# tomasjakab/imm

Measured on AMD Instinct MI355X. Metric: training images/sec at 128x128 K=10, higher is better.
Workload: dtype bf16; 1 GPU; BASELINE configs[1] (N>1: configs[2]): CelebA-shape 128x128 K=10 IMM training step (fwd + VGG16 perceptual loss + bwd + clip + Adam), batch 32 per GPU; global_batch=32, image_size=128, n_maps=10, parallelism=dp1, hip_graph=True, weights=seeded random init; synthetic VGG16 (vgg16.caffemodel.h5 unavailable offline)

## Files before the change

### imm_amd/csrc/conv_wgrad_halo.hip

```cpp
#include "conv_common.h"
#include "conv_dispatch.h"
#include <stdlib.h>
#include <string.h>

typedef __attribute__((ext_vector_type(4))) short s16x4_t;
typedef __attribute__((address_space(3))) s16x4_t lds_s16x4_t;

#ifndef IMM_WH_ABLATE
#define IMM_WH_ABLATE 0
#endif
#define WH_PH 8
#define WH_PW 16
#define WH_HROWS(KH) (WH_PH + (KH) - 1)
#define WH_HCOLS(KW) (WH_PW + (KW) - 1)
#define WH_HP(KH, KW) ((WH_HROWS(KH) * WH_HCOLS(KW) + 63) / 64 * 64)
#define WH_S2_PW 17
#define WH_S2_PP 160
#define WH_S2_HP 640

template <int C8>
__device__ __forceinline__ int wh_swzx(int x) { return C8 == 8 ? ((((x >> 1) & 1) | (((x >> 3) & 1) << 1)) << 1) : (((x >> 3) & 1) << 1); }

struct WgradHaloArgs {
  const uint16_t* x; const uint16_t* dy; float* slab;
  int batch, h, w, ldx, lddy, co, kpad, ci_total;
  int n_patches, patches_x, patches_y;
  int nsplit, nci, nco;
  uint32_t x_bytes, dy_bytes;
  const float* nol_scale; const float* nol_shift; int nol_relu;
};

template <typename ET, int CI, int CO, int NS, int KH = 3, int KW = 3, int ST = 1>
__device__ __forceinline__ void conv_wgrad_halo_body(const WgradHaloArgs& a, const int bx, const int G, const int by, const int bz) {
  static_assert(ST == 1 || (ST == 2 && KH == 3 && KW == 3), "stride 2: 3x3 only");
  constexpr int NTAP = KH * KW, PT = (KH - 1) / 2, PL = (KW - 1) / 2;
  constexpr int WH_HW = WH_HCOLS(KW), HPIX = WH_HROWS(KH) * WH_HCOLS(KW), WH_HP_ = ST == 2 ? WH_S2_HP : WH_HP(KH, KW);
  constexpr int XC8 = CI / 8, YC8 = CO / 8;
  constexpr int NCT = CI / 16, NNT = CO / 16;
  constexpr int WC = NCT, WN = 4 / WC;
  constexpr int TNT = NNT / WN;
  static_assert(WC * WN == 4 && TNT >= 1, "tile split");
  constexpr int X_PIX_PER_DMA = 64 / XC8, Y_PIX_PER_DMA = 64 / YC8;
  constexpr int X_DMA = WH_HP_ / X_PIX_PER_DMA, Y_DMA = 128 / Y_PIX_PER_DMA;
  constexpr int X_BYTES = WH_HP_ * CI * 2, Y_BYTES = 128 * CO * 2, STAGE = X_BYTES + Y_BYTES;
  constexpr int LPP = X_DMA / 4 + Y_DMA / 4;
  static_assert(X_DMA % 4 == 0 && Y_DMA % 4 == 0 && NS >= 2 && (NS - 2) * LPP < 64, "uniform per-wave DMA count");
  extern __shared__ __attribute__((aligned(16))) uint4 smem[];
  const bool nol = a.nol_scale != nullptr;
  float* coef = (float*)((char*)smem + NS * STAGE);

  const int tid = threadIdx.x, lane = tid & 63, wid = tid >> 6;
  const int wc = wid % WC, wn = wid / WC;
  const int ci0 = by * CI, co0 = bz * CO;
  const u32x4_t xr = buffer_rsrc(a.x, a.x_bytes), yr = buffer_rsrc(a.dy, a.dy_bytes);
  const uint32_t lds_base = (uint32_t)(size_t)(lds_void_t*)smem;
  const int per_img = a.patches_x * a.patches_y;

  constexpr int XU = X_DMA / 4, YU = Y_DMA / 4;
  int x_iy[XU], x_ix[XU];
  int x_rel[XU];
  int x_sc[XU];
  uint32_t y_rel[YU];
  const int w_in = ST * a.w, h_in = ST * a.h;
#pragma unroll
  for (int u = 0; u < XU; ++u) {
    const int hp = (wid + 4 * u) * X_PIX_PER_DMA + lane / XC8;
    int iy, ix, col;
    bool valid;
    if constexpr (ST == 2) {
      const int plane = hp / WH_S2_PP, rem = hp - plane * WH_S2_PP;
      const int pi = rem / WH_S2_PW, pj = rem - pi * WH_S2_PW;
      iy = 2 * pi + (plane >> 1); ix = 2 * pj + (plane & 1);
      valid = rem < 9 * WH_S2_PW;
      col = pj;
    } else {
      const int hy = hp / WH_HW, hx = hp - hy * WH_HW;
      iy = hy - PT; ix = hx - PL;
      valid = hp < HPIX;
      col = hx;
    }
    const int sc = (lane % XC8) ^ wh_swzx<XC8>(col);
    x_iy[u] = valid ? iy : (1 << 24);
    x_ix[u] = ix;
    x_rel[u] = ((iy * w_in + ix) * a.ldx + ci0) * 2 + sc * 16;
    x_sc[u] = sc;
  }
  if (nol && tid < CI) {
    coef[(tid >> 3) * 16 + (tid & 7)] = a.nol_scale[ci0 + tid];
    coef[(tid >> 3) * 16 + 8 + (tid & 7)] = a.nol_shift[ci0 + tid];
  }
#pragma unroll
  for (int u = 0; u < YU; ++u) {
    const int p = (wid + 4 * u) * Y_PIX_PER_DMA + lane / YC8;
    const int ty = p >> 4, tx = p & 15;
    const int sc = (lane % YC8) ^ wh_swzx<YC8>(tx);
    y_rel[u] = (uint32_t)(((ty * a.w + tx) * a.lddy + co0) * 2 + sc * 16);
  }

  auto issue = [&](int patch, int stage) {
    const int img = patch / per_img, pr = patch - img * per_img;
    const int y0 = (pr / a.patches_x) * WH_PH, x0 = (pr % a.patches_x) * WH_PW;
    const uint32_t xs = (uint32_t)(img * h_in * w_in) * (uint32_t)(a.ldx * 2);
    const uint32_t ys = (uint32_t)(img * a.h * a.w) * (uint32_t)(a.lddy * 2) + (uint32_t)((y0 * a.w + x0) * a.lddy * 2);
    const int py = ST * y0, px = ST * x0;
    const int poff = (py * w_in + px) * a.ldx * 2;
    const uint32_t lds_stage = lds_base + (uint32_t)(stage * STAGE + wid * 1024);
#pragma unroll
    for (int u = 0; u < XU; ++u) {
      const bool ok = ((unsigned)(py + x_iy[u]) < (unsigned)h_in) && ((unsigned)(px + x_ix[u]) < (unsigned)w_in);
      const uint32_t vo = ok ? (uint32_t)(x_rel[u] + poff) : BUFFER_OOB;
      lds_dma16(xr, __builtin_amdgcn_readfirstlane(lds_stage + (uint32_t)(u * 4096)), vo, xs);
    }
#pragma unroll
    for (int u = 0; u < YU; ++u)
      lds_dma16(yr, __builtin_amdgcn_readfirstlane(lds_stage + (uint32_t)(X_BYTES + u * 4096)), y_rel[u], ys);
  };

  f32x4_t acc[NTAP][TNT];
#pragma unroll
  for (int t = 0; t < NTAP; ++t)
#pragma unroll
    for (int j = 0; j < TNT; ++j) acc[t][j] = f32x4_t{0.f, 0.f, 0.f, 0.f};

  const int i16 = lane & 15, g = lane >> 4;
  const int k_row = g >> 1, k_x = (g & 1) * 8 + (i16 >> 2), ch4 = (i16 & 3) * 4;
  const char* lds_c = (const char*)smem;
  constexpr int KXE = ST == 2 ? 2 : KW;
  const int lx = k_row * (ST == 2 ? WH_S2_PW : WH_HW) + k_x, ly = k_row * WH_PW + k_x;
  uint32_t xb[KXE][2], yb[TNT][2];
#pragma unroll
  for (int e = 0; e < KXE; ++e)
#pragma unroll
    for (int h = 0; h < 2; ++h)
      xb[e][h] = (uint32_t)((lx * XC8 + (((wc * 16 + ch4) >> 3) ^ wh_swzx<XC8>(k_x + e + 4 * h))) * 16 + (ch4 & 4) * 2);
#pragma unroll
  for (int j = 0; j < TNT; ++j)
#pragma unroll
    for (int h = 0; h < 2; ++h)
      yb[j][h] = (uint32_t)(X_BYTES + (ly * YC8 + (((((wn * TNT + j) * 16) + ch4) >> 3) ^ wh_swzx<YC8>(k_x + 4 * h))) * 16 + (ch4 & 4) * 2);

  uint4 af_keep = make_uint4(0, 0, 0, 0);
  const int n_mine = (bx < a.n_patches) ? (a.n_patches - bx + G - 1) / G : 0;
#pragma unroll
  for (int t = 0; t < NS - 1; ++t)
    if (t < n_mine) issue(bx + t * G, t);
  int stage = 0;
  for (int it = 0; it < n_mine; ++it) {
    constexpr int ABL = IMM_WH_ABLATE;
    if (!(ABL & 16) || it == 0) {
      if (it + NS - 2 < n_mine) wait_vmcnt<(NS - 2) * LPP>();
      else wait_vmcnt<0>();
      if (nol) wait_lgkmcnt0();
      __builtin_amdgcn_s_barrier();
    }
    if (it + NS - 1 < n_mine && !(ABL & 1)) {
      int ns = stage + NS - 1; if (ns >= NS) ns -= NS;
      issue(bx + (it + NS - 1) * G, ns);
    }
    const char* Xl = lds_c + stage * STAGE;
    if (nol) {
      const int patch_ = bx + it * G;
      const int img_ = patch_ / per_img, pr_ = patch_ - img_ * per_img;
      const int py_ = ST * (pr_ / a.patches_x) * WH_PH, px_ = ST * (pr_ % a.patches_x) * WH_PW;
      char* Xw = (char*)smem + stage * STAGE + wid * 1024 + lane * 16;
      const bool nrelu = a.nol_relu != 0;
#pragma unroll
      for (int u = 0; u < XU; ++u) {
        if (((unsigned)(py_ + x_iy[u]) < (unsigned)h_in) && ((unsigned)(px_ + x_ix[u]) < (unsigned)w_in)) {
          uint4* slot = (uint4*)(Xw + u * 4096);
          float f[8];
          unpack8<ET>(*slot, f);
          const float4* cf = (const float4*)(coef + x_sc[u] * 16);
          const float4 s0 = cf[0], s1 = cf[1], h0 = cf[2], h1 = cf[3];
          const float sc[8] = {s0.x, s0.y, s0.z, s0.w, s1.x, s1.y, s1.z, s1.w};
          const float sh[8] = {h0.x, h0.y, h0.z, h0.w, h1.x, h1.y, h1.z, h1.w};
#pragma unroll
          for (int e = 0; e < 8; ++e) {
            f[e] = f[e] * sc[e] + sh[e];
            if (nrelu) f[e] = fmaxf(f[e], 0.f);
          }
          *slot = pack8<ET>(f);
        }
      }
      wait_lgkmcnt0();
      __builtin_amdgcn_s_barrier();
    }

    uint4 bfr[4][TNT];
    if (!(ABL & 4) || it == 0)
#pragma unroll
    for (int ks = 0; ks < 4; ++ks)
#pragma unroll
      for (int j = 0; j < TNT; ++j) {
        const s16x4_t lo = __builtin_amdgcn_ds_read_tr16_b64_v4i16((lds_s16x4_t*)(Xl + yb[j][0] + ks * 32 * YC8 * 16));
        const s16x4_t hi = __builtin_amdgcn_ds_read_tr16_b64_v4i16((lds_s16x4_t*)(Xl + yb[j][1] + (ks * 32 + 4) * YC8 * 16));
        const uint2 l2 = __builtin_bit_cast(uint2, lo), h2 = __builtin_bit_cast(uint2, hi);
        bfr[ks][j] = make_uint4(l2.x, l2.y, h2.x, h2.y);
      }
#pragma unroll
    for (int tap = 0; tap < NTAP; ++tap) {
      const int ky = tap / KW, kx = tap % KW;
#pragma unroll
      for (int ks = 0; ks < 4; ++ks) {
        const int e = ST == 2 ? (kx >> 1) : kx;
        const int cp = ST == 2 ? ((ky & 1) * 2 + (kx & 1)) * WH_S2_PP + (ks * 2 + (ky >> 1)) * WH_S2_PW + (kx >> 1)
                               : (ks * 2 + ky) * WH_HW + kx;
        uint4 af;
        if (!(ABL & 2) || (it == 0 && tap == 0 && ks == 0)) {
          const s16x4_t lo = __builtin_amdgcn_ds_read_tr16_b64_v4i16((lds_s16x4_t*)(Xl + xb[e][0] + cp * XC8 * 16));
          const s16x4_t hi = __builtin_amdgcn_ds_read_tr16_b64_v4i16((lds_s16x4_t*)(Xl + xb[e][1] + (cp + 4) * XC8 * 16));
          const uint2 l2 = __builtin_bit_cast(uint2, lo), h2 = __builtin_bit_cast(uint2, hi);
          af = make_uint4(l2.x, l2.y, h2.x, h2.y);
          af_keep = af;
        } else af = af_keep;
        if (!(ABL & 8))
#pragma unroll
        for (int j = 0; j < TNT; ++j) acc[tap][j] = ET::mfma(bfr[ks][j], af, acc[tap][j]);
      }
    }
    if (++stage == NS) stage = 0;
  }

  float* out = a.slab + (int64_t)bx * a.kpad * a.co;
#pragma unroll
  for (int tap = 0; tap < NTAP; ++tap) {
    const int kk = tap * a.ci_total + ci0 + wc * 16 + (lane & 15);
#pragma unroll
    for (int j = 0; j < TNT; ++j) {
      const int n = co0 + (wn * TNT + j) * 16 + 4 * (lane >> 4);
      float* op = out + (int64_t)kk * a.co + n;
      if (IMM_WH_ABLATE & 32) {
        if (acc[tap][j][0] == 123456.789f) op[0] = acc[tap][j][1] + acc[tap][j][2] + acc[tap][j][3];
      } else if (n + 3 < a.co && (a.co & 3) == 0) {
        *(float4*)op = make_float4(acc[tap][j][0], acc[tap][j][1], acc[tap][j][2], acc[tap][j][3]);
      } else {
#pragma unroll
        for (int r = 0; r < 4; ++r) if (n + r < a.co) op[r] = acc[tap][j][r];
      }
    }
  }
}

template <typename ET, int CI, int CO, int NS, int KH = 3, int KW = 3, int ST = 1>
__global__ __launch_bounds__(256) void conv_wgrad_halo_kernel(const WgradHaloArgs a) {
  conv_wgrad_halo_body<ET, CI, CO, NS, KH, KW, ST>(a, blockIdx.x, gridDim.x, blockIdx.y, blockIdx.z);
}

template <typename ET, int CI, int CO, int NS, int KH = 3, int KW = 3, int ST = 1>
__global__ __launch_bounds__(256) void conv_wgrad_halo_multi_kernel(const WgradHaloArgs* __restrict__ tab,
                                                                    const int* __restrict__ first, int n) {
  const int b = blockIdx.x;
  int g = 0;
  while (g + 1 < n && b >= first[g + 1]) ++g;
  const WgradHaloArgs a = tab[g];
  int r = b - first[g];
  const int bx = r % a.nsplit; r /= a.nsplit;
  const int by = r % a.nci, bz = r / a.nci;
  conv_wgrad_halo_body<ET, CI, CO, NS, KH, KW, ST>(a, bx, a.nsplit, by, bz);
}

struct WhPlan { int cs, ns, nci, nco, nsplit; bool k71, s2; };

static bool wh_plan(const imm_conv_desc* d, int lddy, WhPlan* pl) {
  const bool k33 = d->kh == 3 && d->kw == 3 && d->pad_t == 1 && d->pad_l == 1;
  const bool k71 = d->kh == 7 && d->kw == 1 && d->pad_t == 3 && d->pad_l == 0 && d->ci == 32 && lddy == 32 && d->co <= 32;
  pl->k71 = k71;
  const bool s2 = d->kh == 3 && d->kw == 3 && d->stride == 2 && d->pad_t == 0 && d->pad_l == 0 && d->updiv == 1 && d->ci == 32 &&
                  lddy == 64 && d->co > 32 && d->co <= 64 && d->hi == 2 * d->ho && d->wi == 2 * d->wo && d->ho % WH_PH == 0 &&
                  d->wo % WH_PW == 0 && d->ho * d->wo >= 32 * 32 && d->kpad == 9 * d->ci;
  pl->s2 = s2;
  if (s2) {
    const int64_t xb2 = (int64_t)d->batch * d->hi * d->wi * d->ldx * 2, yb2 = (int64_t)d->batch * d->ho * d->wo * lddy * 2;
    if (xb2 >= (1LL << 31) || yb2 >= (1LL << 31)) return false;
    pl->cs = 32; pl->ns = 64; pl->nci = 1; pl->nco = 1;
    const int n_patches2 = d->batch * (d->ho / WH_PH) * (d->wo / WH_PW);
    int ns2 = imm_device_cus();
    if (ns2 > n_patches2 / 4) ns2 = n_patches2 / 4;
    pl->nsplit = ns2 < 1 ? 1 : ns2;
    return true;
  }
  if ((!k33 && !k71) || d->stride != 1 || d->updiv != 1) return false;
  if (d->hi != d->ho || d->wi != d->wo || d->ho % WH_PH || d->wo % WH_PW) return false;
  if (d->kpad != d->kh * d->kw * d->ci || d->ci % 32) return false;
  const int64_t xb = (int64_t)d->batch * d->hi * d->wi * d->ldx * 2, yb = (int64_t)d->batch * d->ho * d->wo * lddy * 2;
  if (xb >= (1LL << 31) || yb >= (1LL << 31)) return false;
  const int n_patches = d->batch * (d->ho / WH_PH) * (d->wo / WH_PW);
  int cs, ns;
  if (d->ci <= 64 && lddy <= 64 && (lddy == 32 || lddy == 64) && d->co <= lddy) {
    if (d->ho * d->wo < 64 * 64) return false;
    cs = d->ci; ns = lddy;
    pl->nci = 1; pl->nco = 1;
  } else {
    if (d->co % 32 || lddy < d->co) return false;
    if (d->ci % 64 == 0 && d->co % 64 == 0 && d->ho * d->wo >= 16 * 16) {
      cs = 64; ns = 64;
    } else {
      if (d->ho * d->wo < 64 * 64) return false;
      cs = 32; ns = 32;
    }
    pl->nci = d->ci / cs; pl->nco = d->co / ns;
  }
  pl->cs = cs; pl->ns = ns;
  const int blocks = pl->nci * pl->nco;
  constexpr int per_cu = 1;
  int grid = per_cu * imm_device_cus();
  if (blocks > 1) grid = imm_device_cus();
  int nsplit = (grid + blocks - 1) / blocks;
  const int min_patches = blocks > 1 ? 2 : 4;
  if (nsplit > n_patches / min_patches) nsplit = n_patches / min_patches;
  if (nsplit < 1) nsplit = 1;
  pl->nsplit = nsplit;
  return true;
}

bool imm_wgrad_halo_applicable(const imm_conv_desc* d, int lddy) {
  static const bool off = imm_conv_disabled("wgrad_halo");
  if (off) return false;
  WhPlan pl;
  return wh_plan(d, lddy, &pl);
}

int imm_wgrad_halo_splits(const imm_conv_desc* d, int lddy) {
  WhPlan pl;
  return wh_plan(d, lddy, &pl) ? pl.nsplit : 0;
}

template <int CI, int CO, int KH, int KW, int ST = 1>
struct WhRing {
  static constexpr int stage = (ST == 2 ? WH_S2_HP : WH_HP(KH, KW)) * CI * 2 + 128 * CO * 2;
  static constexpr int NS = ST == 2 ? 2 : (CI == 32 && CO == 32) ? 3 : (stage > 36 * 1024 ? 3 : 4);
  static constexpr int per_cu = (CI == 32 && CO == 32) ? 2 : 1;
};

template <typename ET, int CI, int CO, int KH = 3, int KW = 3, int ST = 1>
static void wh_launch_cfg(const WgradHaloArgs& a, dim3 grid, hipStream_t s) {
  constexpr int stage = WhRing<CI, CO, KH, KW, ST>::stage;
  constexpr int NS = WhRing<CI, CO, KH, KW, ST>::NS;
  constexpr int lds = NS * stage + CI * 8;
  imm_launch<conv_wgrad_halo_kernel<ET, CI, CO, NS, KH, KW, ST>>(grid, dim3(256), lds, s, a);
}

static WgradHaloArgs wh_fill(const imm_conv_desc* d, const void* x, const void* dy, int lddy, float* slab, int nsplit,
                             const WhPlan& pl, const float* nol_scale = nullptr, const float* nol_shift = nullptr, int nol_relu = 0) {
  WgradHaloArgs a;
  a.nol_scale = nol_scale; a.nol_shift = nol_shift; a.nol_relu = nol_relu;
  a.x = (const uint16_t*)x; a.dy = (const uint16_t*)dy; a.slab = slab;
  a.batch = d->batch; a.h = d->ho; a.w = d->wo; a.ldx = d->ldx; a.lddy = lddy; a.co = d->co; a.kpad = d->kpad;
  a.ci_total = d->ci;
  a.patches_x = d->wo / WH_PW; a.patches_y = d->ho / WH_PH;
  a.n_patches = d->batch * a.patches_x * a.patches_y;
  a.nsplit = nsplit; a.nci = pl.nci; a.nco = pl.nco;
  a.x_bytes = (uint32_t)((int64_t)d->batch * d->hi * d->wi * d->ldx * 2);
  a.dy_bytes = (uint32_t)((int64_t)d->batch * d->ho * d->wo * lddy * 2);
  return a;
}

void imm_wgrad_halo_launch(int dtype, const imm_conv_desc* d, const void* x, const void* dy, int lddy, float* slab,
                           int nsplit, hipStream_t s, const float* nol_scale, const float* nol_shift, int nol_relu) {
  WhPlan pl;
  (void)wh_plan(d, lddy, &pl);
  const WgradHaloArgs a = wh_fill(d, x, dy, lddy, slab, nsplit, pl, nol_scale, nol_shift, nol_relu);
  const dim3 grid(nsplit, pl.nci, pl.nco);
#define WH_GO(ET_) \
  do { \
    if (pl.s2) wh_launch_cfg<ET_, 32, 64, 3, 3, 2>(a, grid, s); \
    else if (pl.k71) wh_launch_cfg<ET_, 32, 32, 7, 1>(a, grid, s); \
    else if (pl.cs == 64 && pl.ns == 64) wh_launch_cfg<ET_, 64, 64>(a, grid, s); \
    else if (pl.cs == 64) wh_launch_cfg<ET_, 64, 32>(a, grid, s); \
    else if (pl.ns == 64) wh_launch_cfg<ET_, 32, 64>(a, grid, s); \
    else wh_launch_cfg<ET_, 32, 32>(a, grid, s); \
  } while (0)
  if (dtype == IMM_BF16) WH_GO(BF16); else WH_GO(F16);
#undef WH_GO
}

int imm_wgrad_halo_variant(const imm_conv_desc* d, int lddy) {
  WhPlan pl;
  return wh_plan(d, lddy, &pl) ? (pl.s2 ? 20000 : pl.k71 ? 7100 : 0) + pl.cs * 100 + pl.ns : 0;
}
int imm_wgrad_halo_blocks(const imm_conv_desc* d, int lddy, int* n_patches) {
  WhPlan pl;
  if (!wh_plan(d, lddy, &pl)) return 0;
  if (n_patches) *n_patches = d->batch * (d->ho / WH_PH) * (d->wo / WH_PW);
  return pl.nci * pl.nco;
}
int imm_wgrad_halo_args_bytes() { return (int)sizeof(WgradHaloArgs); }
int imm_wgrad_halo_fill(const imm_conv_desc* d, const void* x, const void* dy, int lddy, float* slab, int nsplit, void* out,
                        int* steps, const float* nol_scale, const float* nol_shift, int nol_relu) {
  WhPlan pl;
  (void)wh_plan(d, lddy, &pl);
  const WgradHaloArgs a = wh_fill(d, x, dy, lddy, slab, nsplit, pl, nol_scale, nol_shift, nol_relu);
  memcpy(out, &a, sizeof(a));
  if (steps) *steps = (a.n_patches + nsplit - 1) / nsplit * 4 * (pl.cs / 16);
  return nsplit * pl.nci * pl.nco;
}

int imm_wgrad_halo_per_cu(int variant) { return (variant == 3232 || variant == 7100 + 3232) ? 2 : 1; }

template <typename ET, int CI, int CO, int KH = 3, int KW = 3, int ST = 1>
static void wh_launch_multi_cfg(const WgradHaloArgs* tab, const int* first, int n, int blocks, hipStream_t s) {
  constexpr int stage = WhRing<CI, CO, KH, KW, ST>::stage;
  constexpr int NS = WhRing<CI, CO, KH, KW, ST>::NS;
  constexpr int lds = NS * stage + CI * 8;
  imm_launch<conv_wgrad_halo_multi_kernel<ET, CI, CO, NS, KH, KW, ST>>(dim3(blocks), dim3(256), lds, s, tab, first, n);
}

void imm_wgrad_halo_launch_multi(int dtype, int variant, const void* tab_dev, const int* first_dev, int n, int blocks,
                                 hipStream_t s) {
  const WgradHaloArgs* t = (const WgradHaloArgs*)tab_dev;
#define WH_GO(ET_) \
  do { \
    if (variant == 20000 + 3264) wh_launch_multi_cfg<ET_, 32, 64, 3, 3, 2>(t, first_dev, n, blocks, s); \
    else if (variant == 7100 + 3232) wh_launch_multi_cfg<ET_, 32, 32, 7, 1>(t, first_dev, n, blocks, s); \
    else if (variant == 6464) wh_launch_multi_cfg<ET_, 64, 64>(t, first_dev, n, blocks, s); \
    else if (variant == 6432) wh_launch_multi_cfg<ET_, 64, 32>(t, first_dev, n, blocks, s); \
    else if (variant == 3264) wh_launch_multi_cfg<ET_, 32, 64>(t, first_dev, n, blocks, s); \
    else wh_launch_multi_cfg<ET_, 32, 32>(t, first_dev, n, blocks, s); \
  } while (0)
  if (dtype == IMM_BF16) WH_GO(BF16); else WH_GO(F16);
#undef WH_GO
}
```

Before: 10430 images/s.

## Run 64-channel 3x3 wgrad halo kernel with eight waves and row-reuse MFMA schedule

Adds an NW template parameter so the weight-gradient halo kernel can run with 512 threads, splitting the output-channel tiles across eight waves and spreading the DMA rounds over them. For 3x3 stride-1 CI=64 tiles it adds a loop over input halo rows: each transposed LDS read of x is reused across every ky tap it feeds, and a short prefetch ring plus sched_group_barrier pinning interleaves ds_reads with MFMAs. The aim is more latency hiding and fewer redundant LDS reads per MFMA, at the cost of fewer accumulator tiles per wave and extra barrier and sync cost across twice as many waves. It also adds an exported probe entry point for the 64x64 variant.

```diff
diff --git a/imm_amd/csrc/conv_wgrad_halo.hip b/imm_amd/csrc/conv_wgrad_halo.hip
--- a/imm_amd/csrc/conv_wgrad_halo.hip
+++ b/imm_amd/csrc/conv_wgrad_halo.hip
@@ -8,6 +8,9 @@
 
 #ifndef IMM_WH_ABLATE
 #define IMM_WH_ABLATE 0
+#endif
+#ifndef IMM_WH_WAVES8
+#define IMM_WH_WAVES8 3
 #endif
 #define WH_PH 8
 #define WH_PW 16
@@ -21,6 +24,12 @@
 template <int C8>
 __device__ __forceinline__ int wh_swzx(int x) { return C8 == 8 ? ((((x >> 1) & 1) | (((x >> 3) & 1) << 1)) << 1) : (((x >> 3) & 1) << 1); }
 
+constexpr int wh_uses(int r, int kh) {
+  int n = 0;
+  for (int ky = 0; ky < kh; ++ky) n += (r - ky >= 0 && ((r - ky) & 1) == 0 && (r - ky) / 2 < 4) ? 1 : 0;
+  return n;
+}
+
 struct WgradHaloArgs {
   const uint16_t* x; const uint16_t* dy; float* slab;
   int batch, h, w, ldx, lddy, co, kpad, ci_total;
@@ -30,21 +39,22 @@
   const float* nol_scale; const float* nol_shift; int nol_relu;
 };
 
-template <typename ET, int CI, int CO, int NS, int KH = 3, int KW = 3, int ST = 1>
+template <typename ET, int CI, int CO, int NS, int KH = 3, int KW = 3, int ST = 1, int NW = 4>
 __device__ __forceinline__ void conv_wgrad_halo_body(const WgradHaloArgs& a, const int bx, const int G, const int by, const int bz) {
   static_assert(ST == 1 || (ST == 2 && KH == 3 && KW == 3), "stride 2: 3x3 only");
   constexpr int NTAP = KH * KW, PT = (KH - 1) / 2, PL = (KW - 1) / 2;
   constexpr int WH_HW = WH_HCOLS(KW), HPIX = WH_HROWS(KH) * WH_HCOLS(KW), WH_HP_ = ST == 2 ? WH_S2_HP : WH_HP(KH, KW);
   constexpr int XC8 = CI / 8, YC8 = CO / 8;
   constexpr int NCT = CI / 16, NNT = CO / 16;
-  constexpr int WC = NCT, WN = 4 / WC;
+  static_assert(NW == 4 || NW == 8, "four or eight waves");
+  constexpr int WC = NCT, WN = NW / WC;
   constexpr int TNT = NNT / WN;
-  static_assert(WC * WN == 4 && TNT >= 1, "tile split");
+  static_assert(WC * WN == NW && TNT >= 1 && TNT * WN == NNT, "tile split");
   constexpr int X_PIX_PER_DMA = 64 / XC8, Y_PIX_PER_DMA = 64 / YC8;
   constexpr int X_DMA = WH_HP_ / X_PIX_PER_DMA, Y_DMA = 128 / Y_PIX_PER_DMA;
   constexpr int X_BYTES = WH_HP_ * CI * 2, Y_BYTES = 128 * CO * 2, STAGE = X_BYTES + Y_BYTES;
-  constexpr int LPP = X_DMA / 4 + Y_DMA / 4;
-  static_assert(X_DMA % 4 == 0 && Y_DMA % 4 == 0 && NS >= 2 && (NS - 2) * LPP < 64, "uniform per-wave DMA count");
+  constexpr int LPP = X_DMA / NW + Y_DMA / NW;
+  static_assert(X_DMA % NW == 0 && Y_DMA % NW == 0 && NS >= 2 && (NS - 2) * LPP < 64, "uniform per-wave DMA count");
   extern __shared__ __attribute__((aligned(16))) uint4 smem[];
   const bool nol = a.nol_scale != nullptr;
   float* coef = (float*)((char*)smem + NS * STAGE);
@@ -56,7 +66,8 @@
   const uint32_t lds_base = (uint32_t)(size_t)(lds_void_t*)smem;
   const int per_img = a.patches_x * a.patches_y;
 
-  constexpr int XU = X_DMA / 4, YU = Y_DMA / 4;
+  constexpr int XU = X_DMA / NW, YU = Y_DMA / NW;
+  constexpr int ROUND = NW * 1024;
   int x_iy[XU], x_ix[XU];
   int x_rel[XU];
   int x_sc[XU];
@@ -64,7 +75,7 @@
   const int w_in = ST * a.w, h_in = ST * a.h;
 #pragma unroll
   for (int u = 0; u < XU; ++u) {
-    const int hp = (wid + 4 * u) * X_PIX_PER_DMA + lane / XC8;
+    const int hp = (wid + NW * u) * X_PIX_PER_DMA + lane / XC8;
     int iy, ix, col;
     bool valid;
     if constexpr (ST == 2) {
@@ -91,7 +102,7 @@
   }
 #pragma unroll
   for (int u = 0; u < YU; ++u) {
-    const int p = (wid + 4 * u) * Y_PIX_PER_DMA + lane / YC8;
+    const int p = (wid + NW * u) * Y_PIX_PER_DMA + lane / YC8;
     const int ty = p >> 4, tx = p & 15;
     const int sc = (lane % YC8) ^ wh_swzx<YC8>(tx);
     y_rel[u] = (uint32_t)(((ty * a.w + tx) * a.lddy + co0) * 2 + sc * 16);
@@ -109,11 +120,11 @@
     for (int u = 0; u < XU; ++u) {
       const bool ok = ((unsigned)(py + x_iy[u]) < (unsigned)h_in) && ((unsigned)(px + x_ix[u]) < (unsigned)w_in);
       const uint32_t vo = ok ? (uint32_t)(x_rel[u] + poff) : BUFFER_OOB;
-      lds_dma16(xr, __builtin_amdgcn_readfirstlane(lds_stage + (uint32_t)(u * 4096)), vo, xs);
+      lds_dma16(xr, __builtin_amdgcn_readfirstlane(lds_stage + (uint32_t)(u * ROUND)), vo, xs);
     }
 #pragma unroll
     for (int u = 0; u < YU; ++u)
-      lds_dma16(yr, __builtin_amdgcn_readfirstlane(lds_stage + (uint32_t)(X_BYTES + u * 4096)), y_rel[u], ys);
+      lds_dma16(yr, __builtin_amdgcn_readfirstlane(lds_stage + (uint32_t)(X_BYTES + u * ROUND)), y_rel[u], ys);
   };
 
   f32x4_t acc[NTAP][TNT];
@@ -167,7 +178,7 @@
 #pragma unroll
       for (int u = 0; u < XU; ++u) {
         if (((unsigned)(py_ + x_iy[u]) < (unsigned)h_in) && ((unsigned)(px_ + x_ix[u]) < (unsigned)w_in)) {
-          uint4* slot = (uint4*)(Xw + u * 4096);
+          uint4* slot = (uint4*)(Xw + u * ROUND);
           float f[8];
           unpack8<ET>(*slot, f);
           const float4* cf = (const float4*)(coef + x_sc[u] * 16);
@@ -197,6 +208,39 @@
         const uint2 l2 = __builtin_bit_cast(uint2, lo), h2 = __builtin_bit_cast(uint2, hi);
         bfr[ks][j] = make_uint4(l2.x, l2.y, h2.x, h2.y);
       }
+    if constexpr (NW == 8 && ST == 1) {
+      constexpr int NR = WH_HROWS(KH), NF = NR * KW, PD = 3;
+      auto xread = [&](int f) {
+        const int cp = (f / KW) * WH_HW + f % KW;
+        if ((ABL & 2) && !(it == 0 && f == 0)) return af_keep;
+        const s16x4_t lo = __builtin_amdgcn_ds_read_tr16_b64_v4i16((lds_s16x4_t*)(Xl + xb[f % KW][0] + cp * XC8 * 16));
+        const s16x4_t hi = __builtin_amdgcn_ds_read_tr16_b64_v4i16((lds_s16x4_t*)(Xl + xb[f % KW][1] + (cp + 4) * XC8 * 16));
+        const uint2 l2 = __builtin_bit_cast(uint2, lo), h2 = __builtin_bit_cast(uint2, hi);
+        return make_uint4(l2.x, l2.y, h2.x, h2.y);
+      };
+      uint4 ar[PD + 1];
+#pragma unroll
+      for (int f = 0; f < PD; ++f) ar[f] = xread(f);
+      if (ABL & 2) af_keep = ar[0];
+      constexpr bool PIN = (ABL & (2 | 4 | 8)) == 0;
+      if constexpr (PIN) __builtin_amdgcn_sched_group_barrier(SG_DSREAD, 8 * TNT + 2 * PD, 0);
+      static_for<0, NF>([&](auto F) {
+        constexpr int f = decltype(F)::value, r = f / KW, kx = f % KW;
+        if constexpr (f + PD < NF) ar[(f + PD) % (PD + 1)] = xread(f + PD);
+        const uint4 af = ar[f % (PD + 1)];
+        constexpr int n_mfma = (ABL & 8) ? 0 : TNT * wh_uses(r, KH);
+#pragma unroll
+        for (int ky = 0; ky < KH; ++ky) {
+          const int d = r - ky;
+          if (d >= 0 && (d & 1) == 0 && d / 2 < 4 && !(ABL & 8)) {
+#pragma unroll
+            for (int j = 0; j < TNT; ++j) acc[ky * KW + kx][j] = ET::mfma(bfr[d / 2][j], af, acc[ky * KW + kx][j]);
+          }
+        }
+        if constexpr (PIN && f + PD < NF) __builtin_amdgcn_sched_group_barrier(SG_DSREAD, 2, 0);
+        if constexpr (PIN && n_mfma > 0) __builtin_amdgcn_sched_group_barrier(SG_MFMA, n_mfma, 0);
+      });
+    } else
 #pragma unroll
     for (int tap = 0; tap < NTAP; ++tap) {
       const int ky = tap / KW, kx = tap % KW;
@@ -241,14 +285,14 @@
   }
 }
 
-template <typename ET, int CI, int CO, int NS, int KH = 3, int KW = 3, int ST = 1>
-__global__ __launch_bounds__(256) void conv_wgrad_halo_kernel(const WgradHaloArgs a) {
-  conv_wgrad_halo_body<ET, CI, CO, NS, KH, KW, ST>(a, blockIdx.x, gridDim.x, blockIdx.y, blockIdx.z);
-}
-
-template <typename ET, int CI, int CO, int NS, int KH = 3, int KW = 3, int ST = 1>
-__global__ __launch_bounds__(256) void conv_wgrad_halo_multi_kernel(const WgradHaloArgs* __restrict__ tab,
-                                                                    const int* __restrict__ first, int n) {
+template <typename ET, int CI, int CO, int NS, int KH = 3, int KW = 3, int ST = 1, int NW = 4>
+__global__ __launch_bounds__(NW * 64) void conv_wgrad_halo_kernel(const WgradHaloArgs a) {
+  conv_wgrad_halo_body<ET, CI, CO, NS, KH, KW, ST, NW>(a, blockIdx.x, gridDim.x, blockIdx.y, blockIdx.z);
+}
+
+template <typename ET, int CI, int CO, int NS, int KH = 3, int KW = 3, int ST = 1, int NW = 4>
+__global__ __launch_bounds__(NW * 64) void conv_wgrad_halo_multi_kernel(const WgradHaloArgs* __restrict__ tab,
+                                                                       const int* __restrict__ first, int n) {
   const int b = blockIdx.x;
   int g = 0;
   while (g + 1 < n && b >= first[g + 1]) ++g;
@@ -256,7 +300,7 @@
   int r = b - first[g];
   const int bx = r % a.nsplit; r /= a.nsplit;
   const int by = r % a.nci, bz = r / a.nci;
-  conv_wgrad_halo_body<ET, CI, CO, NS, KH, KW, ST>(a, bx, a.nsplit, by, bz);
+  conv_wgrad_halo_body<ET, CI, CO, NS, KH, KW, ST, NW>(a, bx, a.nsplit, by, bz);
 }
 
 struct WhPlan { int cs, ns, nci, nco, nsplit; bool k71, s2; };
@@ -330,6 +374,8 @@
   static constexpr int stage = (ST == 2 ? WH_S2_HP : WH_HP(KH, KW)) * CI * 2 + 128 * CO * 2;
   static constexpr int NS = ST == 2 ? 2 : (CI == 32 && CO == 32) ? 3 : (stage > 36 * 1024 ? 3 : 4);
   static constexpr int per_cu = (CI == 32 && CO == 32) ? 2 : 1;
+  static constexpr int NW = (KH == 3 && KW == 3 && ST == 1 && CI == 64 &&
+                             ((CO == 64 && (IMM_WH_WAVES8 & 1)) || (CO == 32 && (IMM_WH_WAVES8 & 2)))) ? 8 : 4;
 };
 
 template <typename ET, int CI, int CO, int KH = 3, int KW = 3, int ST = 1>
@@ -337,7 +383,8 @@
   constexpr int stage = WhRing<CI, CO, KH, KW, ST>::stage;
   constexpr int NS = WhRing<CI, CO, KH, KW, ST>::NS;
   constexpr int lds = NS * stage + CI * 8;
-  imm_launch<conv_wgrad_halo_kernel<ET, CI, CO, NS, KH, KW, ST>>(grid, dim3(256), lds, s, a);
+  constexpr int NW = WhRing<CI, CO, KH, KW, ST>::NW;
+  imm_launch<conv_wgrad_halo_kernel<ET, CI, CO, NS, KH, KW, ST, NW>>(grid, dim3(NW * 64), lds, s, a);
 }
 
 static WgradHaloArgs wh_fill(const imm_conv_desc* d, const void* x, const void* dy, int lddy, float* slab, int nsplit,
@@ -402,7 +449,8 @@
   constexpr int stage = WhRing<CI, CO, KH, KW, ST>::stage;
   constexpr int NS = WhRing<CI, CO, KH, KW, ST>::NS;
   constexpr int lds = NS * stage + CI * 8;
-  imm_launch<conv_wgrad_halo_multi_kernel<ET, CI, CO, NS, KH, KW, ST>>(dim3(blocks), dim3(256), lds, s, tab, first, n);
+  constexpr int NW = WhRing<CI, CO, KH, KW, ST>::NW;
+  imm_launch<conv_wgrad_halo_multi_kernel<ET, CI, CO, NS, KH, KW, ST, NW>>(dim3(blocks), dim3(NW * 64), lds, s, tab, first, n);
 }
 
 void imm_wgrad_halo_launch_multi(int dtype, int variant, const void* tab_dev, const int* first_dev, int n, int blocks,
@@ -420,3 +468,23 @@
   if (dtype == IMM_BF16) WH_GO(BF16); else WH_GO(F16);
 #undef WH_GO
 }
+
+extern "C" int imm_wgrad_halo_probe6464(const imm_conv_desc* d, int dtype, const void* x, const void* dy, int lddy, float* slab,
+                                        int nsplit, const float* x_scale, const float* x_shift, int x_relu, void* stream) {
+  IMM_REQUIRE(d && x && dy && slab && nsplit >= 1 && (dtype == IMM_BF16 || dtype == IMM_F16), "wgrad_halo_probe6464: args");
+  IMM_REQUIRE(d->kh == 3 && d->kw == 3 && d->pad_t == 1 && d->pad_l == 1 && d->stride == 1 && d->updiv == 1 && d->hi == d->ho &&
+              d->wi == d->wo && d->ho % WH_PH == 0 && d->wo % WH_PW == 0, "wgrad_halo_probe6464: 3x3 stride 1 on whole 8x16 patches");
+  IMM_REQUIRE(d->ci % 64 == 0 && d->co % 64 == 0 && d->kpad == 9 * d->ci && d->ldx >= d->ci && d->ldx % 8 == 0 && lddy >= d->co &&
+              lddy % 8 == 0, "wgrad_halo_probe6464: channels");
+  IMM_REQUIRE((x_scale == nullptr) == (x_shift == nullptr), "wgrad_halo_probe6464: x_scale / x_shift come together");
+  IMM_REQUIRE((int64_t)d->batch * d->hi * d->wi * d->ldx * 2 < (1LL << 31) && (int64_t)d->batch * d->ho * d->wo * lddy * 2 < (1LL << 31),
+              "wgrad_halo_probe6464: operand beyond a 32-bit buffer extent");
+  WhPlan pl;
+  pl.cs = 64; pl.ns = 64; pl.nci = d->ci / 64; pl.nco = d->co / 64; pl.nsplit = nsplit; pl.k71 = false; pl.s2 = false;
+  const WgradHaloArgs a = wh_fill(d, x, dy, lddy, slab, nsplit, pl, x_scale, x_shift, x_relu);
+  const dim3 grid(nsplit, pl.nci, pl.nco);
+  if (dtype == IMM_BF16) wh_launch_cfg<BF16, 64, 64>(a, grid, (hipStream_t)stream);
+  else wh_launch_cfg<F16, 64, 64>(a, grid, (hipStream_t)stream);
+  IMM_CHECK_LAUNCH("imm_wgrad_halo_probe6464");
+  return 0;
+}
```

Result: no change. 10500 images/s, median of 6 (+0.6%).
